# takahiroharada/OCLRadixSort

Hardware: AMD Instinct MI355X
Metric: Gkeys/s on uniform-random u32 keys; achieved % of HBM-read roofline (higher is better)
Workload: dtype u32; 1 GPU; Key-only RadixSort32, 67108864 uniform-random u32 keys (splitmix64 hi32, seed 123+step), 1xMI355X, in place; keys_per_gpu=67108864, parallelism=1 GPU, sort_algo=auto, digit_bits=8

## Files before the change

oclradixsort_amd/csrc/adlhip.hip:

```cpp
#include "../../include/adlhip.h"

#include <hip/hip_runtime.h>

#include <algorithm>
#include <cmath>
#include <cstdarg>
#include <cstdio>
#include <cstdlib>
#include <cstring>
#include <map>
#include <mutex>
#include <utility>
#include <string>
#include <vector>

#include "radix_kernels.hpp"
#include "onesweep_kernels.hpp"
#include "hybrid_kernels.hpp"
#include "persist_kernels.hpp"
#include "finish16_kernels.hpp"
#include "soa_wide_kernels.hpp"
#include "typed_kernels.hpp"

#ifndef ADLHIP_SINGLE_TU
#define X(...) extern template __global__ __VA_ARGS__;
#include "finish_kernels.inc"
#include "wavefinish_kernels.inc"
#include "passes_kernels.inc"
#include "perdigit_kernels.inc"
#undef X
#endif

namespace {

thread_local char g_err[512] = "";

int fail(const char* fmt, ...)
{
    va_list ap;
    va_start(ap, fmt);
    vsnprintf(g_err, sizeof(g_err), fmt, ap);
    va_end(ap);
    if (getenv("ADLHIP_VERBOSE")) fprintf(stderr, "[adlhip] error: %s\n", g_err);
    return ADLHIP_FAILURE;
}

#define HIPCHK(expr)                                                                           \
    do {                                                                                       \
        hipError_t _e = (expr);                                                                \
        if (_e != hipSuccess)                                                                  \
            return fail("%s failed: %s (%s:%d)", #expr, hipGetErrorString(_e), __FILE__, __LINE__); \
    } while (0)

struct ProfEntry {
    uint64_t launches = 0;
    double total_ms = 0.0;
};
struct PendingProf {
    const char* name;
    hipEvent_t e0, e1;
};
struct Staging {
    void* hptr;
    size_t bytes;
    hipEvent_t done;
    size_t capacity;
};
struct PinnedBlock {
    void* hptr;
    size_t capacity;
};
constexpr size_t kPinnedPoolMax = size_t(512) << 20;

}

struct adlhip_event {
    hipEvent_t ev;
};

struct adlhip_device {
    int idx = 0;
    hipStream_t stream = nullptr;
    bool own_stream = true;
    hipDeviceProp_t prop;
    uint64_t used_bytes = 0;
    int sort_algo = -1;
    int digit_bits = 8;
    int profile = 0;
    int tile_variant = -1;
    int rank_mode = 1;
    int lds_ordered = 0;
    int resident_wgs_device = 0;
    int resident_wgs = 0;
    int mid_path = 1;
    int mid_skip = 0;
    int mid2_skip = 0;
    int mid_backoff = 32, mid2_backoff = 64;
    int bin_finish = 1;
    int persist = 1;
    int msd2_path = 1;
    int net_lookback = 1;
    int partition_lookback = 1;
    int dict_path = 1;
    adlhip::DictBlock* d_dict = nullptr;
    uint32_t* d_msd2 = nullptr;
    std::vector<PendingProf> pending;
    std::vector<hipEvent_t> event_pool;
    std::map<std::string, ProfEntry> prof;
    std::vector<std::string> prof_order;
    std::vector<Staging> staging;
    std::vector<PinnedBlock> pinned_pool;
    size_t pinned_pool_bytes = 0;
    uint32_t* d_fault = nullptr;
    uint32_t* h_fault = nullptr;
    hipEvent_t fault_snap = nullptr;
    uint32_t* d_mid_hist = nullptr;
};

namespace {

int bind(adlhip_device* d)
{
    if (!d) return fail("null device handle");
    HIPCHK(hipSetDevice(d->idx));
    return ADLHIP_SUCCESS;
}

hipEvent_t take_event(adlhip_device* d)
{
    if (!d->event_pool.empty()) {
        hipEvent_t e = d->event_pool.back();
        d->event_pool.pop_back();
        return e;
    }
    hipEvent_t e = nullptr;
    if (hipEventCreate(&e) != hipSuccess) return nullptr;
    return e;
}

inline int trace_level()
{
    static const int level = getenv("ADLHIP_TRACE") ? atoi(getenv("ADLHIP_TRACE")) : 0;
    return level;
}

template <typename F>
int launch(adlhip_device* d, const char* name, F&& f)
{
    hipEvent_t e0 = nullptr, e1 = nullptr;
    if (d->profile) {
        e0 = take_event(d);
        e1 = take_event(d);
        if (!e0 || !e1) return fail("hipEventCreate failed");
        HIPCHK(hipEventRecord(e0, d->stream));
    }
    static const int trace = trace_level();
    if (trace) fprintf(stderr, "[adlhip] launch %s\n", name), fflush(stderr);
    f();
    hipError_t e = hipGetLastError();
    if (e != hipSuccess) return fail("launch of %s failed: %s", name, hipGetErrorString(e));
    if (trace == 1 && (e = hipStreamSynchronize(d->stream)) != hipSuccess) return fail("%s: %s", name, hipGetErrorString(e));
    if (d->profile) {
        HIPCHK(hipEventRecord(e1, d->stream));
        d->pending.push_back({name, e0, e1});
    }
    return ADLHIP_SUCCESS;
}

int fold_profile(adlhip_device* d)
{
    if (d->pending.empty()) return ADLHIP_SUCCESS;
    HIPCHK(hipStreamSynchronize(d->stream));
    for (auto& p : d->pending) {
        float ms = 0.f;
        HIPCHK(hipEventElapsedTime(&ms, p.e0, p.e1));
        auto it = d->prof.find(p.name);
        if (it == d->prof.end()) {
            d->prof_order.push_back(p.name);
            it = d->prof.emplace(p.name, ProfEntry()).first;
        }
        it->second.launches++;
        it->second.total_ms += ms;
// ... 868 lines not shown
    if (total > region_bytes || (size_t)passes * rows * 256 * 4 >= (size_t(1) << 31)) return os;
    os.ctrl = reinterpret_cast<adlhip::u32x4*>(region);
    os.tables = reinterpret_cast<adlhip::PassTable*>(region + off_tables);
    os.joint = reinterpret_cast<uint32_t*>(region + off_joint);
    os.part = reinterpret_cast<uint32_t*>(region + off_part);
    os.status = reinterpret_cast<uint32_t*>(region + off_status);
    os.rows = (uint32_t)rows;
    os.hist_wgs = wgs;
    os.per_wg = per_wg;
    os.slice0 = per_wg * wgs_per_slice;
    return os;
}

Msd2Layout msd2_layout(size_t n, size_t elem_bytes, int headroom_pct = kFullHeadroomPct)
{
    Msd2Layout L;
    const uint32_t tile = elem_bytes == 4 ? 16384u : 8192u;
    static const int env_pct = getenv("ADLHIP_SLAB_A_HEADROOM_PCT") ? atoi(getenv("ADLHIP_SLAB_A_HEADROOM_PCT")) : -1;
    if (headroom_pct == kFullHeadroomPct && env_pct >= 0) headroom_pct = env_pct;
    L.stride_a = (uint32_t)align_up(n / 256 + (n / 256) * (size_t)headroom_pct / 100 + 4096, 64);
    L.seg_shift = msd2_seg_shift(n, elem_bytes == 8);
    L.slots = 256u << L.seg_shift;
    const bool fine = elem_bytes == 4 && L.seg_shift == 8;
    L.stride_b = msd2_stride_b(n, L.slots, fine);
    L.tier_b = msd2_tier_b(n, L.slots, fine);
    L.tiles_per_bucket = (L.stride_a + tile - 1) / tile;
    L.off_mode = 0;
    L.off_cnt = L.off_mode + 256;
    L.off_off = L.off_cnt + 65536 * 4;
    L.off_hard = align_up(L.off_off + 65537 * 4, 256);
    L.off_coop = L.off_hard + 65536 * 4;
    L.off_slab_a = align_up(L.off_coop + kNetTableBytes, 256);
    L.off_slab_b = align_up(L.off_slab_a + (size_t)256 * L.stride_a * elem_bytes, 256);
    const size_t slab_b_bytes = (size_t)L.slots * L.stride_b * (elem_bytes == 4 && L.seg_shift == 8 ? 2 : elem_bytes);
    L.slab_b_in_tmp = elem_bytes == 4 && L.seg_shift == 8 && n >= kSlabInTmpMin && slab_b_bytes <= n * elem_bytes;
    L.total = L.off_slab_b + (L.slab_b_in_tmp ? 0 : slab_b_bytes);
    return L;
}

template <typename E, typename S, bool SOA = false>
int launch_large_finish(adlhip_device* d, const E* slab_b, E* out, uint32_t* out_vals, uint32_t* seg_off, uint32_t* seg_cnt, uint32_t stride_b,
                        uint32_t tier_b, uint32_t* mode, uint32_t* hard, int low_bits_max, bool bin, uint32_t seg_shift = 8);
bool use_bin_finish(const adlhip_device* d, size_t elem_bytes, bool key64, size_t n, bool whole_keys);

template <typename E>
int msd2_sort(adlhip_device* d, E* data, E* tmp, void* work, size_t n, int headroom_pct = kFullHeadroomPct)
{
    constexpr int K = sizeof(E) == 4 ? 32 : 16;
    constexpr int KEY_BITS = 8 * (int)sizeof(E);
    constexpr bool k32 = sizeof(E) == 4;
    uint32_t* cur_a = d->d_msd2;
    uint32_t* cur_b = d->d_msd2 + 8192;
    uint32_t* flag = d->d_msd2 + 8192 + 65536;
    uint32_t* done = flag + 1;
    uint32_t* sample = flag + 8;
    const Msd2Layout L = msd2_layout(n, sizeof(E), headroom_pct);
    char* wb = reinterpret_cast<char*>(work);
    uint32_t* mode = reinterpret_cast<uint32_t*>(wb + L.off_mode);
    uint32_t* seg_cnt = reinterpret_cast<uint32_t*>(wb + L.off_cnt);
    uint32_t* seg_off = reinterpret_cast<uint32_t*>(wb + L.off_off);
    E* slab_a = reinterpret_cast<E*>(wb + L.off_slab_a);
    E* slab_b = L.slab_b_in_tmp ? tmp : reinterpret_cast<E*>(wb + L.off_slab_b);
    using CT = adlhip::TileCfg<E, 8, 512, K>;
    auto kern = adlhip::msd_bucket_scatter_kernel<E, 512, K, 1>;
    auto kern2 = adlhip::msd_bucket_scatter_kernel<E, 512, K, 2>;
    if (ensure_lds(kern, CT::LDS_BYTES) || ensure_lds(kern2, CT::LDS_BYTES)) return ADLHIP_FAILURE;
    int rc = launch(d, "msd2_sample", [&] {
        hipLaunchKernelGGL(adlhip::msd2_sample_kernel<E>, dim3(adlhip::kSampleWGs), dim3(64), 0, d->stream, (const E*)data, (uint32_t)n,
                           sample, flag + 2, d->d_fault, flag, sample_dup_threshold(n));
    });
    if (rc) return rc;
    adlhip::BucketPass<E> pa;
    pa.src = data; pa.dst = slab_a; pa.cursors = cur_a; pa.cursor_shift = 5; pa.src_count_shift = 0; pa.flag = flag;
    pa.src_counts = nullptr; pa.n = (uint32_t)n;
    pa.src_stride = 0; pa.tiles_per_bucket = 1; pa.dst_stride = L.stride_a; pa.dst_total = 256u * L.stride_a; pa.start_bit = KEY_BITS - 8;
    pa.zero_me = nullptr; pa.sample = sample; pa.which_digit = 1; pa.dst16 = 0;
    pa.place = nullptr; pa.status_a = nullptr; pa.pieces = 0; pa.rows_per_chain_a = 0; pa.slice = 0; pa.seg_shift = 8;
    const uint32_t tiles_a = (uint32_t)((n + CT::TILE - 1) / CT::TILE);
    const bool slab16 = sizeof(E) == 4 && L.seg_shift == 8;
    const bool persist = d->persist && (size_t)256 * L.stride_a * sizeof(E) < (size_t(1) << 32) - (1u << 20) &&
                         (size_t)L.slots * L.stride_b * (slab16 ? 2 : sizeof(E)) < (size_t(1) << 32) - (1u << 20);
    using PC = adlhip::PersistCfg<E, 512, K>;
    const uint32_t pgrid = (uint32_t)(2 * d->prop.multiProcessorCount + 7) / 8 * 8;
    if (persist) {
        auto pk = adlhip::msd_scatter_persist_kernel<E, 512, K, 1, 4, false, 2, 0>;
        if (ensure_lds(pk, PC::LDS_BYTES)) return ADLHIP_FAILURE;
        rc = launch(d, k32 ? "msd2_pass1_u32" : "msd2_pass1_u64", [&] { hipLaunchKernelGGL(pk, dim3(pgrid), dim3(512), PC::LDS_BYTES, d->stream, pa); });
    } else {
        rc = launch(d, k32 ? "msd2_pass1_u32" : "msd2_pass1_u64", [&] { hipLaunchKernelGGL(kern, dim3(tiles_a), dim3(512), CT::LDS_BYTES, d->stream, pa); });
    }
    if (rc) return rc;
    adlhip::BucketPass<E> pb = pa;
    pb.src = slab_a; pb.dst = slab_b; pb.cursors = cur_b; pb.cursor_shift = 0; pb.src_count_shift = 5; pb.flag = flag;
    pb.src_counts = cur_a; pb.n = (uint32_t)n;
    pb.src_stride = L.stride_a; pb.tiles_per_bucket = L.tiles_per_bucket; pb.dst_stride = L.stride_b;
    pb.dst_total = L.slots * L.stride_b; pb.start_bit = KEY_BITS - 16; pb.zero_me = nullptr;
    pb.sample = sample; pb.which_digit = 2; pb.seg_shift = L.seg_shift;
    pb.dst16 = slab16 ? 1 : 0;
    if (persist) {
        auto pk16 = adlhip::msd_scatter_persist_kernel<E, 512, K, 2, 4, true, 2, 0>;
        auto pkE = adlhip::msd_scatter_persist_kernel<E, 512, K, 2, 4, false, 2, 0>;
        if (ensure_lds(pk16, PC::LDS_BYTES) || ensure_lds(pkE, PC::LDS_BYTES)) return ADLHIP_FAILURE;
        rc = launch(d, k32 ? "msd2_pass2_u32" : "msd2_pass2_u64", [&] {
            if (slab16) hipLaunchKernelGGL(pk16, dim3(pgrid), dim3(512), PC::LDS_BYTES, d->stream, pb);
            else hipLaunchKernelGGL(pkE, dim3(pgrid), dim3(512), PC::LDS_BYTES, d->stream, pb);
        });
    } else {
        rc = launch(d, k32 ? "msd2_pass2_u32" : "msd2_pass2_u64", [&] {
            hipLaunchKernelGGL(kern2, dim3(256 * L.tiles_per_bucket), dim3(512), CT::LDS_BYTES, d->stream, pb);
        });
    }
    if (rc) return rc;
    uint32_t* bar = done + 1;
    uint32_t* ctable = reinterpret_cast<uint32_t*>(wb + L.off_coop);
    using CC = adlhip::TileCfg<E, 8, 512, K>;
    auto ko = adlhip::msd2_offsets_kernel<E, 512, K>;
    if (ensure_lds(ko, CC::LDS_BYTES)) return ADLHIP_FAILURE;
    rc = launch(d, "msd2_offsets", [&] {
        hipLaunchKernelGGL(ko, dim3(net_wgs(d)), dim3(512), CC::LDS_BYTES, d->stream, cur_a, cur_b, flag, done, bar,
                           seg_cnt, seg_off, mode, (uint32_t)n, sample, data, tmp, ctable, d->d_fault, KEY_BITS,
                           8u - L.seg_shift, d->dict_path ? d->d_dict : nullptr, net_stats(d),
                           net_onesweep_args(d, wb + L.off_slab_a, (size_t)256 * L.stride_a * sizeof(E), n, 4, CC::TILE));
    });
    if (rc) return rc;
    using S = typename std::conditional<sizeof(E) == 4, uint16_t, E>::type;
    uint32_t* hard = reinterpret_cast<uint32_t*>(wb + L.off_hard);
    const int low_max = KEY_BITS - 8 - (int)L.seg_shift;
    const bool bin = use_bin_finish(d, sizeof(E), sizeof(E) == 8, L.seg_shift < 8 ? (size_t(24) << 20) : n, true);
    if (sizeof(E) == 4 && !slab16)
        return launch_large_finish<E, E>(d, slab_b, data, nullptr, seg_off, seg_cnt, L.stride_b, L.tier_b, mode, hard, low_max, bin, L.seg_shift);
    return launch_large_finish<E, S>(d, slab_b, data, nullptr, seg_off, seg_cnt, L.stride_b, L.tier_b, mode, hard, low_max, bin, L.seg_shift);
}

constexpr size_t kMsd2sAutoMin = size_t(1) << 20;
constexpr size_t kMsd2sMax = (size_t(1) << 28) + (size_t(1) << 22);
constexpr uint32_t msd2s_tile(size_t elem_bytes) { return elem_bytes == 8 ? 8192u : 16384u; }

struct Msd2sLayout {
    size_t off_mode, off_place, off_cnt, off_off, off_hard, off_coop, off_tickets, off_status_a, off_status_b, off_slab_a, off_slab_b, total;
    uint32_t pieces, slice, rows_a, rows_b, stride_a, stride_b, tier_b, ticket_words, seg_shift, slots;
    size_t status_bytes_a, status_bytes_b;
    bool slab_b_in_tmp;
};

Msd2sLayout msd2s_layout(size_t n, size_t elem_bytes = 8, bool slab16 = false, bool lean = false)
{
    Msd2sLayout L;
    const uint32_t kMsd2sTile = msd2s_tile(elem_bytes);
    double best = 1e30;
    for (uint32_t p : {16u}) {
        const size_t slice = align_up((n + p - 1) / p, kMsd2sTile);
        const size_t mean = slice / 256;
        size_t sd = 1;
        while (sd * sd < mean) ++sd;
        const size_t stride = align_up(mean + (lean ? 0 : mean / 2) + 8 * sd + 64, 64);
        const double waste = (double)((stride + kMsd2sTile - 1) / kMsd2sTile) * kMsd2sTile / (double)mean;
        if (waste < best - 1e-9) {
            best = waste;
            L.pieces = p;
            L.slice = (uint32_t)slice;
            L.stride_a = (uint32_t)stride;
        }
    }
    L.rows_a = L.slice / kMsd2sTile;
    L.rows_b = (uint32_t)(((size_t)L.pieces * L.stride_a + kMsd2sTile - 1) / kMsd2sTile);
    L.seg_shift = slab16 ? 8u : msd2_seg_shift(n, false);
    L.slots = 256u << L.seg_shift;
    L.stride_b = msd2_stride_b(n, L.slots, slab16, lean);
    L.tier_b = msd2_tier_b(n, L.slots, slab16);
    L.ticket_words = (32 + 256) * adlhip::kTicketStride;
    L.status_bytes_a = (size_t)L.pieces * L.rows_a * 1024;
    L.status_bytes_b = (size_t)256 * L.rows_b * 1024;
    L.off_mode = 0;
    L.off_place = 128;
    L.off_cnt = 256;
    L.off_off = L.off_cnt + 65536 * 4;
    L.off_hard = align_up(L.off_off + 65537 * 4, 256);
    L.off_coop = L.off_hard + 65536 * 4;
    L.off_tickets = align_up(L.off_coop + kNetTableBytes, 256);
    size_t sdb = 1;
    while (sdb * sdb * 4096 < n) ++sdb;
    const size_t bucket_bound = n / 256 + (lean ? 0 : n / 512) + 24 * (32 + 16 + 8 * (sdb + 1) + 128);
    const size_t rows_a_bound = n / kMsd2sTile + 24;
    const size_t rows_b_bound = bucket_bound / kMsd2sTile + 25;
// ... 1322 lines not shown
        });
        if (rc) return rc;
        rc = launch(d, "scan_partials", [&] {
            hipLaunchKernelGGL(adlhip::scan_single_kernel, dim3(1), dim3(adlhip::kScanNT), 0, d->stream,
                               (const uint32_t*)partial, partial, blocks, d_total);
        });
        if (rc) return rc;
        rc = launch(d, "scan_apply", [&] {
            hipLaunchKernelGGL(adlhip::scan_apply_kernel, dim3((uint32_t)blocks), dim3(adlhip::kScanNT), 0, d->stream,
                               src, dst, (const uint32_t*)partial, n);
        });
        if (rc) return rc;
    }
    if (h_sum) HIPCHK(hipMemcpyAsync(h_sum, d_total, 4, hipMemcpyDeviceToHost, d->stream));
    return ADLHIP_SUCCESS;
}


int adlhip_partition_msb_u32(adlhip_device* d, const uint32_t* in, uint32_t* out, uint32_t* counts, void* work,
                             size_t work_bytes, size_t n, int num_buckets)
{
    return partition_msb<uint32_t>(d, in, out, counts, work, work_bytes, n, num_buckets);
}

int adlhip_partition_msb_kv32(adlhip_device* d, const void* in, void* out, uint32_t* counts, void* work, size_t work_bytes,
                              size_t n, int num_buckets)
{
    return partition_msb<uint64_t>(d, static_cast<const uint64_t*>(in), static_cast<uint64_t*>(out), counts, work, work_bytes, n,
                                   num_buckets);
}

int adlhip_partition_top_byte_u32(adlhip_device* d, const uint32_t* in, uint32_t* out, uint32_t* totals256, void* work,
                                  size_t work_bytes, size_t n)
{
    return partition_top_byte_entry<uint32_t>(d, in, out, totals256, work, work_bytes, n);
}

int adlhip_partition_top_byte_kv32(adlhip_device* d, const void* in, void* out, uint32_t* totals256, void* work,
                                   size_t work_bytes, size_t n)
{
    return partition_top_byte_entry<uint64_t>(d, static_cast<const uint64_t*>(in), static_cast<uint64_t*>(out), totals256, work,
                                              work_bytes, n);
}


int adlhip_generate_keys(adlhip_device* d, int elem_kind, void* dptr, size_t n, uint64_t seed, uint64_t first_index)
{
    if (bind(d)) return ADLHIP_FAILURE;
    if (elem_kind < ADLHIP_ELEM_U32 || elem_kind > ADLHIP_ELEM_U64) return fail("bad element kind %d", elem_kind);
    if (n == 0) return ADLHIP_SUCCESS;
    if (!dptr) return fail("null buffer");
    const uint64_t base = seed * 0x9E3779B97F4A7C15ull + first_index;
    const int grid = (int)std::min<size_t>((n + 255) / 256, (size_t)d->prop.multiProcessorCount * 16);
    return launch(d, "generate_keys", [&] {
        hipLaunchKernelGGL(adlhip::generate_keys_kernel, dim3(grid), dim3(256), 0, d->stream, dptr, n, base, first_index, elem_kind);
    });
}


int adlhip_set_param(adlhip_device* d, const char* name, int value)
{
    if (!d || !name) return fail("null argument");
    if (!strcmp(name, "sort.algo")) {
        if (value < -1 || value > 1) return fail("sort.algo must be -1, 0 or 1");
        d->sort_algo = value;
    } else if (!strcmp(name, "sort.digit_bits")) {
        if (value != 4 && value != 7 && value != 8) return fail("sort.digit_bits must be 4, 7 or 8");
        d->digit_bits = value;
    } else if (!strcmp(name, "sort.tile")) {
        if (value < -1 || value >= kNumVariants) return fail("sort.tile must be in [-1,%d)", kNumVariants);
        d->tile_variant = value;

    } else if (!strcmp(name, "sort.mid")) {
        if (value < 0 || value > 3) return fail("sort.mid must be 0 (off), 1 (on), 2 (keys: always the two-launch form) or 3 (always the three-launch form)");
        d->mid_path = value;
    } else if (!strcmp(name, "sort.msd2")) {
        if (value < 0 || value > 5)
            return fail("sort.msd2 must be 0 (off), 1 (on), 2 (always, from 1 Mi elements; forms by size), 3 (always the stable passes), "
                        "4 (always the cursor passes for whole keys) or 5 (always the hybrid form for whole keys)");
        d->msd2_path = value;
    } else if (!strcmp(name, "sort.persist")) {
        if (value != 0 && value != 1) return fail("sort.persist must be 0 (one tile per workgroup, round 3) or 1 (persistent prefetching passes + 16-bit finish)");
        d->persist = value;
    } else if (!strcmp(name, "sort.net_lookback")) {
        d->net_lookback = value ? 1 : 0;
    } else if (!strcmp(name, "partition.lookback")) {
        d->partition_lookback = value ? 1 : 0;
    } else if (!strcmp(name, "sort.dict")) {
        if (value != 0 && value != 1) return fail("sort.dict must be 0 (off) or 1 (counting sort for keys that take few distinct values)");
        d->dict_path = value;
    } else if (!strcmp(name, "sort.binfinish")) {
        if (value < 0 || value > 2) return fail("sort.binfinish must be 0 (LSD finish), 1 (binning finish for whole u64 keys from 24 Mi keys up) or 2 (always, u32 keys too)");
        d->bin_finish = value;
    } else if (!strcmp(name, "debug.resident_wgs")) {
        if (value < 0) return fail("debug.resident_wgs must be >= 0");
        d->resident_wgs = value ? value : d->resident_wgs_device;
    } else if (!strcmp(name, "debug.idle_poke")) {
        const int region = (int)((uint32_t)value >> 24);
        const uint32_t word = (uint32_t)value & 0xffffffu;
        if (region < 1 || region > kIdleRegions || word >= idle_region_words(region))
            return fail("debug.idle_poke: no word %u in region %d (region << 24 | word; regions 1 d_msd2, 2 d_mid_hist, 3 d_dict, 4 d_fault)", word, region);
        if (bind(d)) return ADLHIP_FAILURE;
        hipLaunchKernelGGL(idle_poke_kernel, dim3(1), dim3(1), 0, d->stream, idle_region_base(d, region) + word);
        HIPCHK(hipGetLastError());
    } else if (!strcmp(name, "sort.rank")) {
        if (value != 0 && value != 1) return fail("sort.rank must be 0 or 1");
        if (value == 1 && !d->lds_ordered) return fail("sort.rank = 1 needs lane-ordered DS atomics; the device self-test failed");
        d->rank_mode = value;
    } else if (!strcmp(name, "profile")) {
        if (bind(d)) return ADLHIP_FAILURE;
        if (!value && fold_profile(d)) return ADLHIP_FAILURE;
        d->profile = value ? 1 : 0;
    } else {
        return fail("unknown parameter '%s'", name);
    }
    return ADLHIP_SUCCESS;
}

int adlhip_get_param(adlhip_device* d, const char* name, int* value)
{
    if (!d || !name || !value) return fail("null argument");
    if (!strcmp(name, "sort.algo")) *value = d->sort_algo;
    else if (!strcmp(name, "sort.digit_bits")) *value = d->digit_bits;
    else if (!strcmp(name, "sort.tile")) *value = d->tile_variant;
    else if (!strcmp(name, "sort.rank")) *value = d->rank_mode;
    else if (!strcmp(name, "sort.mid")) *value = d->mid_path;
    else if (!strcmp(name, "sort.msd2")) *value = d->msd2_path;
    else if (!strcmp(name, "sort.binfinish")) *value = d->bin_finish;
    else if (!strcmp(name, "sort.persist")) *value = d->persist;
    else if (!strcmp(name, "sort.dict")) *value = d->dict_path;
    else if (!strcmp(name, "partition.lookback")) *value = d->partition_lookback;
    else if (!strcmp(name, "sort.net_lookback")) *value = d->net_lookback;
    else if (!strcmp(name, "debug.resident_wgs")) *value = d->resident_wgs;
    else if (!strcmp(name, "stat.net_runs") || !strcmp(name, "stat.net_counting")) {
        uint32_t v[2] = {0u, 0u};
        HIPCHK(hipMemcpyAsync(v, net_stats(d), 8, hipMemcpyDeviceToHost, d->stream));
        HIPCHK(hipStreamSynchronize(d->stream));
        *value = (int)v[name[9] == 'c' ? 1 : 0];
    }
    else if (!strcmp(name, "debug.idle_dirty") || !strcmp(name, "debug.idle_first")) {
        uint32_t dirty = 0u, first = 0u;
        if (idle_check(d, &dirty, &first)) return ADLHIP_FAILURE;
        *value = (int)(name[11] == 'd' ? dirty : first);
    }
    else if (!strncmp(name, "debug.net_stamp", 15) && name[15] >= '0' && name[15] <= '9' && !name[16]) {
        uint32_t v = 0u;
        HIPCHK(hipMemcpyAsync(&v, net_stats(d) + 4 + (name[15] - '0'), 4, hipMemcpyDeviceToHost, d->stream));
        HIPCHK(hipStreamSynchronize(d->stream));
        *value = (int)(v & 0x7fffffffu);
    }
    else if (!strcmp(name, "sort.lds_ordered")) *value = d->lds_ordered;
    else if (!strcmp(name, "profile")) *value = d->profile;
    else return fail("unknown parameter '%s'", name);
    return ADLHIP_SUCCESS;
}


int adlhip_event_create(adlhip_device* d, adlhip_event** out)
{
    if (bind(d)) return ADLHIP_FAILURE;
    if (!out) return fail("null out pointer");
    adlhip_event* e = new adlhip_event();
    if (hipEventCreate(&e->ev) != hipSuccess) {
        delete e;
        return fail("hipEventCreate failed");
    }
    *out = e;
    return ADLHIP_SUCCESS;
}

int adlhip_event_record(adlhip_device* d, adlhip_event* ev)
{
    if (bind(d)) return ADLHIP_FAILURE;
    if (!ev) return fail("null event");
    HIPCHK(hipEventRecord(ev->ev, d->stream));
    return ADLHIP_SUCCESS;
}

int adlhip_event_elapsed_ms(adlhip_device* d, adlhip_event* a, adlhip_event* b, float* ms)
{
    if (bind(d)) return ADLHIP_FAILURE;
    if (!a || !b || !ms) return fail("null argument");
    HIPCHK(hipEventSynchronize(b->ev));
    HIPCHK(hipEventElapsedTime(ms, a->ev, b->ev));
    return ADLHIP_SUCCESS;
}

int adlhip_event_synchronize(adlhip_device* d, adlhip_event* ev)
{
    if (bind(d)) return ADLHIP_FAILURE;
    if (!ev) return fail("null event");
    HIPCHK(hipEventSynchronize(ev->ev));
    return ADLHIP_SUCCESS;
}

int adlhip_event_query(adlhip_device* d, adlhip_event* ev, int* done)
{
    if (bind(d)) return ADLHIP_FAILURE;
    if (!ev || !done) return fail("null argument");
    const hipError_t e = hipEventQuery(ev->ev);
    if (e != hipSuccess && e != hipErrorNotReady) return fail("hipEventQuery failed: %s", hipGetErrorString(e));
    (void)hipGetLastError();
    *done = e == hipSuccess ? 1 : 0;
    return ADLHIP_SUCCESS;
}

int adlhip_event_destroy(adlhip_device* d, adlhip_event* ev)
{
    if (bind(d)) return ADLHIP_FAILURE;
    if (!ev) return ADLHIP_SUCCESS;
    hipEventDestroy(ev->ev);
    delete ev;
// ... 116 lines not shown
```

oclradixsort_amd/csrc/passes_kernels.inc:

```
X(void adlhip::msd2_offsets_kernel<unsigned int, 512, 32>(unsigned int*, unsigned int*, unsigned int*, unsigned int*, unsigned int*, unsigned int*, unsigned int*, unsigned int*, unsigned int, unsigned int*, unsigned int*, unsigned int*, unsigned int*, unsigned int*, int, unsigned int, adlhip::DictBlock*, unsigned int*, adlhip::OsNet))
X(void adlhip::msd2_offsets_kernel<unsigned long, 512, 16>(unsigned int*, unsigned int*, unsigned int*, unsigned int*, unsigned int*, unsigned int*, unsigned int*, unsigned int*, unsigned int, unsigned int*, unsigned long*, unsigned long*, unsigned int*, unsigned int*, int, unsigned int, adlhip::DictBlock*, unsigned int*, adlhip::OsNet))
X(void adlhip::msd2s_offsets_kernel<unsigned int, 16384, 512, 32, 1, 4>(unsigned int const*, unsigned int, unsigned int, unsigned int, unsigned int const*, unsigned int, unsigned int, unsigned int*, unsigned int*, unsigned int*, unsigned int*, unsigned int*, unsigned int*, unsigned int, adlhip::StablePlace const*, unsigned int*, unsigned int*, unsigned int*, unsigned int*, unsigned int*, unsigned int*, unsigned int*, unsigned int, adlhip::DictBlock*, unsigned int*, adlhip::OsNet))
X(void adlhip::msd2s_offsets_kernel<unsigned long, 8192, 512, 16, 0, 4>(unsigned int const*, unsigned int, unsigned int, unsigned int, unsigned int const*, unsigned int, unsigned int, unsigned int*, unsigned int*, unsigned int*, unsigned int*, unsigned int*, unsigned int*, unsigned int, adlhip::StablePlace const*, unsigned long*, unsigned long*, unsigned int*, unsigned int*, unsigned int*, unsigned int*, unsigned int*, unsigned int, adlhip::DictBlock*, unsigned int*, adlhip::OsNet))
X(void adlhip::msd2s_offsets_kernel<unsigned long, 8192, 512, 16, 1, 4>(unsigned int const*, unsigned int, unsigned int, unsigned int, unsigned int const*, unsigned int, unsigned int, unsigned int*, unsigned int*, unsigned int*, unsigned int*, unsigned int*, unsigned int*, unsigned int, adlhip::StablePlace const*, unsigned long*, unsigned long*, unsigned int*, unsigned int*, unsigned int*, unsigned int*, unsigned int*, unsigned int, adlhip::DictBlock*, unsigned int*, adlhip::OsNet))
X(void adlhip::msd2s_offsets_kernel<unsigned long, 8192, 512, 16, 1, 8>(unsigned int const*, unsigned int, unsigned int, unsigned int, unsigned int const*, unsigned int, unsigned int, unsigned int*, unsigned int*, unsigned int*, unsigned int*, unsigned int*, unsigned int*, unsigned int, adlhip::StablePlace const*, unsigned long*, unsigned long*, unsigned int*, unsigned int*, unsigned int*, unsigned int*, unsigned int*, unsigned int, adlhip::DictBlock*, unsigned int*, adlhip::OsNet))
X(void adlhip::msd_bucket_scatter_kernel<unsigned int, 256, 16, 0>(adlhip::BucketPass<unsigned int>))
X(void adlhip::msd_bucket_scatter_kernel<unsigned int, 512, 32, 1>(adlhip::BucketPass<unsigned int>))
X(void adlhip::msd_bucket_scatter_kernel<unsigned int, 512, 32, 2>(adlhip::BucketPass<unsigned int>))
X(void adlhip::msd_bucket_scatter_kernel<unsigned int, 512, 32, 3>(adlhip::BucketPass<unsigned int>))
X(void adlhip::msd_bucket_scatter_kernel<unsigned long, 512, 16, 1>(adlhip::BucketPass<unsigned long>))
X(void adlhip::msd_bucket_scatter_kernel<unsigned long, 512, 16, 2>(adlhip::BucketPass<unsigned long>))
X(void adlhip::msd_bucket_scatter_kernel<unsigned long, 512, 16, 3>(adlhip::BucketPass<unsigned long>))
X(void adlhip::msd_lookback_scatter_kernel<unsigned int, 512, 32, false, 1>(adlhip::LookbackPass<unsigned int>))
X(void adlhip::msd_lookback_scatter_kernel<unsigned long, 512, 16, false, 0>(adlhip::LookbackPass<unsigned long>))
X(void adlhip::msd_lookback_scatter_kernel<unsigned long, 512, 16, false, 1>(adlhip::LookbackPass<unsigned long>))
X(void adlhip::msd_lookback_scatter_kernel<unsigned long, 512, 16, true, 1>(adlhip::LookbackPass<unsigned long>))
X(void adlhip::msd_scatter_persist_kernel<unsigned int, 512, 32, 1, 4, false, 2, 0>(adlhip::BucketPass<unsigned int>))
X(void adlhip::msd_scatter_persist_kernel<unsigned int, 512, 32, 2, 4, false, 2, 0>(adlhip::BucketPass<unsigned int>))
X(void adlhip::msd_scatter_persist_kernel<unsigned int, 512, 32, 2, 4, true, 2, 0>(adlhip::BucketPass<unsigned int>))
X(void adlhip::msd_scatter_persist_kernel<unsigned long, 512, 16, 1, 4, false, 2, 0>(adlhip::BucketPass<unsigned long>))
X(void adlhip::msd_scatter_persist_kernel<unsigned long, 512, 16, 2, 4, false, 2, 0>(adlhip::BucketPass<unsigned long>))
X(void adlhip::msd_scatter_persist_kernel<unsigned long, 512, 16, 2, 4, true, 2, 0>(adlhip::BucketPass<unsigned long>))
```

oclradixsort_amd/csrc/persist_kernels.hpp:

```cpp
#pragma once
#include <hip/hip_runtime.h>
#include <stdint.h>

#include "hybrid_kernels.hpp"

namespace adlhip {

template <typename E, int NT, int K>
struct PersistCfg {
    static constexpr int NW = NT / 64;
    static constexpr int TILE = NT * K;
    static constexpr int VEC = 16 / (int)sizeof(E);
    static_assert(K % VEC == 0, "whole 16-byte loads");
    static_assert(TILE <= 65536, "16-bit tile positions");
    static constexpr size_t OFF_ELEMS = 0;
    static constexpr size_t OFF_WCNT = sizeof(E) * TILE;
    static constexpr size_t OFF_WPOS = OFF_WCNT + sizeof(uint32_t) * NW * 256;
    static constexpr size_t OFF_GOFF = OFF_WPOS + sizeof(uint16_t) * NW * 256;
    static constexpr size_t OFF_PREF = OFF_GOFF + sizeof(uint32_t) * 256;
    static constexpr size_t OFF_BCNT = OFF_PREF + sizeof(uint32_t) * 260;
    static constexpr size_t OFF_WSUM = OFF_BCNT + sizeof(uint32_t) * 256;
    static constexpr size_t LDS_BYTES = OFF_WSUM + 64;
};

struct PersistTile {
    uint32_t base;
    uint32_t valid;
    uint32_t cursor_base;
};

template <typename E, int B>
__device__ __forceinline__ void rank_batch(const E* e, uint32_t* rnk, uint32_t* my_wcnt, int start_bit)
{
    const uint32_t dg0 = digit_of<8>(e[0], start_bit);
    const uint32_t d0 = (uint32_t)__builtin_amdgcn_readfirstlane((int)dg0);
    bool same = false;
    if (__all(dg0 == d0)) {
        same = true;
#pragma unroll
        for (int j = 1; j < B; ++j) same &= digit_of<8>(e[j], start_bit) == d0;
    }
    const uint32_t left = (uint32_t)__builtin_amdgcn_update_dpp((int)~dg0, (int)dg0, 0x111, 0xf, 0xf, false);
    const bool few_runs = __popcll(__ballot(left != dg0)) <= 8;
    const bool dominant = __popcll(__ballot(dg0 == d0)) >= 40;
    const int peel = few_runs ? 4 : (dominant ? 1 : 0);
    if (__all(same)) {
        uint32_t old = 0u;
        if (lane_id() == 0) old = __hip_atomic_fetch_add(&my_wcnt[d0], (uint32_t)(64 * B), __ATOMIC_RELAXED, __HIP_MEMORY_SCOPE_WORKGROUP);
        old = (uint32_t)__builtin_amdgcn_readfirstlane((int)old);
#pragma unroll
        for (int j = 0; j < B; ++j) rnk[j] = old + (uint32_t)(j * 64 + lane_id());
    } else if (peel) {
#pragma unroll
        for (int j = 0; j < B; ++j) {
            const uint32_t d = digit_of<8>(e[j], start_bit);
            uint64_t todo = __ballot(true);
            uint32_t r = 0u;
#pragma unroll 1
            for (int it = 0; it < peel && todo; ++it) {
                const uint64_t m0 = few_runs ? todo : __ballot(d == d0);
                if (!m0) break;
                const int lead = __builtin_ctzll(m0);
                const uint32_t dl = (uint32_t)__builtin_amdgcn_readlane((int)d, lead);
                const uint64_t m = __ballot(d == dl);
                uint32_t old = 0u;
                if (lane_id() == lead)
                    old = __hip_atomic_fetch_add(&my_wcnt[dl], (uint32_t)__popcll(m), __ATOMIC_RELAXED, __HIP_MEMORY_SCOPE_WORKGROUP);
                old = (uint32_t)__builtin_amdgcn_readlane((int)old, lead);
                if (d == dl) r = old + mbcnt64(m);
                todo &= ~m;
            }
            if ((todo >> lane_id()) & 1ull) r = __hip_atomic_fetch_add(&my_wcnt[d], 1u, __ATOMIC_RELAXED, __HIP_MEMORY_SCOPE_WORKGROUP);
            rnk[j] = r;
        }
    } else {
#pragma unroll
        for (int j = 0; j < B; ++j)
            rnk[j] = __hip_atomic_fetch_add(&my_wcnt[digit_of<8>(e[j], start_bit)], 1u, __ATOMIC_RELAXED, __HIP_MEMORY_SCOPE_WORKGROUP);
    }
}

template <typename E, int NT, int K, int PASS, int WPE, bool D16, int LAUX = 0, int SAUX = 0>
__global__ __launch_bounds__(NT, WPE) void msd_scatter_persist_kernel(BucketPass<E> a)
{
    using C = PersistCfg<E, NT, K>;
    constexpr int NW = C::NW;
    constexpr int TILE = C::TILE;
    constexpr int VEC = C::VEC;
    constexpr int Q = K / VEC;
    extern __shared__ __attribute__((aligned(16))) unsigned char smem[];
    E* __restrict__ s_elems = reinterpret_cast<E*>(smem + C::OFF_ELEMS);
    uint32_t* __restrict__ s_wcnt = reinterpret_cast<uint32_t*>(smem + C::OFF_WCNT);
    uint32_t* __restrict__ s_goff = reinterpret_cast<uint32_t*>(smem + C::OFF_GOFF);
    uint32_t* __restrict__ s_pref = reinterpret_cast<uint32_t*>(smem + C::OFF_PREF);
    uint32_t* __restrict__ s_bcnt = reinterpret_cast<uint32_t*>(smem + C::OFF_BCNT);
    const int tid = (int)threadIdx.x;
    const int lane = tid & 63;
    const int w = tid >> 6;
    if (a.zero_me && blockIdx.x == 0 && tid == 0) __hip_atomic_store(a.zero_me, 0u, __ATOMIC_RELAXED, __HIP_MEMORY_SCOPE_AGENT);

    uint32_t* __restrict__ s_give = reinterpret_cast<uint32_t*>(smem + C::OFF_WSUM);
    {
        if (tid == 0) s_give[8] = large_sort_gave_up(a.flag);
        __syncthreads();
        if (s_give[8]) return;
        __syncthreads();
    }
    int start_bit = a.start_bit;
    Msd2Placement place{0, 0ull};
    if (a.sample) {
        place = msd2_placement(a.sample);
        start_bit = place.top - 8 * a.which_digit;
    }
    if constexpr (PASS >= 2) start_bit += 8 - (int)a.seg_shift;

    const uint32_t G = gridDim.x, g = blockIdx.x;
    uint32_t ticket, t_end, t_step, t_origin = 0u;
    if constexpr (PASS == 1) {
        ticket = g;
        t_end = (a.n + (uint32_t)TILE - 1u) / (uint32_t)TILE;
        t_step = G;
    } else {
        uint32_t* s_wsum = reinterpret_cast<uint32_t*>(smem + C::OFF_WSUM);
        uint32_t tiles = 0u;
        if (tid < 256) {
            const uint32_t b = (((uint32_t)tid & 31u) << 3) | ((uint32_t)tid >> 5);
            uint32_t cnt = a.src_counts[b << a.src_count_shift];
            if (cnt > a.src_stride) cnt = a.src_stride;
            s_bcnt[tid] = cnt;
            tiles = (cnt + (uint32_t)TILE - 1u) / (uint32_t)TILE;
        }
        uint32_t total;
        const uint32_t ex = block_excl_scan_u32<NT>(tiles, s_wsum, &total);
        if (tid < 256) s_pref[tid] = ex;
        if (tid == 0) s_pref[256] = total;
        __syncthreads();
        const uint32_t x = g & 7u;
        t_origin = 32u * x;
        ticket = s_pref[t_origin] + (g >> 3);
        t_end = s_pref[t_origin + 32u];
        t_step = G >> 3;
    }
    if (ticket >= t_end) return;

    auto tile_of = [&](uint32_t t) -> PersistTile {
        PersistTile r;
        if constexpr (PASS == 1) {
            r.base = t * (uint32_t)TILE;
            const uint32_t left = a.n - r.base;
            r.valid = left < (uint32_t)TILE ? left : (uint32_t)TILE;
            r.cursor_base = 0u;
        } else {
            uint32_t p = t_origin;
#pragma unroll
            for (uint32_t s = 16u; s >= 1u; s >>= 1)
                if (s_pref[p + s] <= t) p += s;
            const uint32_t b = ((p & 31u) << 3) | (p >> 5);
            const uint32_t off = (t - s_pref[p]) * (uint32_t)TILE;
            const uint32_t room = s_bcnt[p] - off;
            r.base = b * a.src_stride + off;
            r.valid = room < (uint32_t)TILE ? room : (uint32_t)TILE;
            r.cursor_base = b * 256u;
        }
        return r;
    };
    const uint32_t wbase0 = (uint32_t)(w * 64 * K + lane * VEC);
    auto load_tile = [&](const PersistTile& t, E(&e)[K]) {
        uint32_t wbase = wbase0;
        asm volatile("" : "+v"(wbase));
        const __amdgpu_buffer_rsrc_t r = __builtin_amdgcn_make_buffer_rsrc(const_cast<E*>(a.src + (size_t)t.base), 0,
                                                                           (int)(t.valid * (uint32_t)sizeof(E)), 0x00020000);
        const int off = (int)(wbase * (uint32_t)sizeof(E));
#pragma unroll
        for (int q = 0; q < Q; ++q) {
            const u32x4 v = __builtin_amdgcn_raw_buffer_load_b128(r, off, q * 64 * 16, LAUX);
            if constexpr (VEC == 4) {
                e[q * 4 + 0] = v.x; e[q * 4 + 1] = v.y; e[q * 4 + 2] = v.z; e[q * 4 + 3] = v.w;
            } else {
                e[q * 2 + 0] = (E)v.x | ((E)v.y << 32);
                e[q * 2 + 1] = (E)v.z | ((E)v.w << 32);
            }
        }
    };

    uint32_t* my_wcnt = s_wcnt + w * 256;
    uint16_t* __restrict__ my_wpos = reinterpret_cast<uint16_t*>(smem + C::OFF_WPOS) + w * 256;
    constexpr uint32_t SC = D16 ? 2u : (uint32_t)sizeof(E);
    const __amdgpu_buffer_rsrc_t dst_rsrc = __builtin_amdgcn_make_buffer_rsrc(a.dst, 0, (int)(a.dst_total * SC), 0x00020000);

    E cur[K], nxt[K];
    PersistTile tc = tile_of(ticket), tn{0u, 0u, 0u};
    load_tile(tc, cur);
#pragma unroll
    for (int j = 0; j < K; ++j) asm volatile("" : "+v"(cur[j]));
    uint32_t flag_prev = 0u;
    for (;;) {
        const uint32_t ticket_n = ticket + t_step;
        const bool has_next = ticket_n < t_end;
        const uint32_t flag_now = __hip_atomic_load(a.flag, __ATOMIC_RELAXED, __HIP_MEMORY_SCOPE_AGENT);
        if (has_next) {
            tn = tile_of(ticket_n);
            load_tile(tn, nxt);
        }
        const uint32_t valid = tc.valid;
        const bool full = valid == (uint32_t)TILE;
        uint32_t tid_v = (uint32_t)tid;
        asm volatile("" : "+v"(tid_v));
        const uint32_t wbase = (tid_v >> 6) * (uint32_t)(64 * K) + (tid_v & 63u) * (uint32_t)VEC;
        const int rem = (int)valid - (int)wbase;
        if (PASS == 1 && a.sample && place.top < (int)(8 * sizeof(E))) {
            const E pre = (E)place.prefix;
            E bad = E(0);
#pragma unroll
            for (int q = 0; q < Q; ++q)
#pragma unroll
                for (int c = 0; c < VEC; ++c)
                    if (full || q * 64 * VEC + c < rem) bad |= (cur[q * VEC + c] >> place.top) ^ pre;
            if (bad != E(0)) __hip_atomic_fetch_or(a.flag, 1u, __ATOMIC_RELAXED, __HIP_MEMORY_SCOPE_AGENT);
        }
#pragma unroll
        for (int b = lane; b < 256; b += 64) my_wcnt[b] = 0u;
        uint32_t rnk2[(K + 1) / 2];
        if (full) {
            constexpr int B = 8;
            static_assert(K % B == 0, "whole batches");
#pragma unroll
            for (int j0 = 0; j0 < K; j0 += B) {
                uint32_t rnk[B];
                rank_batch<E, B>(cur + j0, rnk, my_wcnt, start_bit);
#pragma unroll
                for (int j = 0; j < B; j += 2) rnk2[(j0 + j) >> 1] = rnk[j] | (rnk[j + 1] << 16);
            }
        } else {
#pragma unroll
            for (int j = 0; j < K; j += 2) {
                uint32_t r0 = 0u, r1 = 0u;
                if ((j / VEC) * 64 * VEC + (j % VEC) < rem)
                    r0 = __hip_atomic_fetch_add(&my_wcnt[digit_of<8>(cur[j], start_bit)], 1u, __ATOMIC_RELAXED, __HIP_MEMORY_SCOPE_WORKGROUP);
                if (((j + 1) / VEC) * 64 * VEC + ((j + 1) % VEC) < rem)
                    r1 = __hip_atomic_fetch_add(&my_wcnt[digit_of<8>(cur[j + 1], start_bit)], 1u, __ATOMIC_RELAXED, __HIP_MEMORY_SCOPE_WORKGROUP);
                rnk2[j >> 1] = r0 | (r1 << 16);
            }
        }
#pragma unroll
        for (int j = 0; j < (K + 1) / 2; ++j) asm volatile("" : "+v"(rnk2[j]));
        if (lane == 0) s_give[w] = flag_prev;
        lds_barrier();
        {
            const u32x4 g0 = *reinterpret_cast<const u32x4*>(s_give), g1 = *reinterpret_cast<const u32x4*>(s_give + 4);
            static_assert(NW <= 8, "one word per wave");
            uint32_t any = 0u;
            if (NW > 0) any |= g0.x; if (NW > 1) any |= g0.y; if (NW > 2) any |= g0.z; if (NW > 3) any |= g0.w;
            if (NW > 4) any |= g1.x; if (NW > 5) any |= g1.y; if (NW > 6) any |= g1.z; if (NW > 7) any |= g1.w;
            if (any) break;
        }
        u32x4 cnt4 = {0u, 0u, 0u, 0u};
        u32x4 toff4 = {0u, 0u, 0u, 0u};
        {
            u32x4 pre4 = {0u, 0u, 0u, 0u};
#pragma unroll
            for (int i = 0; i < NW; ++i) {
                const u32x4 r = *reinterpret_cast<const u32x4*>(s_wcnt + i * 256 + 4 * lane);
                cnt4 += r;
                if (i < w) pre4 += r;
            }
            const uint32_t s4 = cnt4.x + cnt4.y + cnt4.z + cnt4.w;
            const uint32_t ex = wave_incl_scan_u32(s4) - s4;
            toff4.x = ex;
            toff4.y = ex + cnt4.x;
            toff4.z = toff4.y + cnt4.y;
            toff4.w = toff4.z + cnt4.z;
            const u32x4 p4 = toff4 + pre4;
            typedef uint32_t u32x2 __attribute__((ext_vector_type(2)));
            const u32x2 packed = {p4.x | (p4.y << 16), p4.z | (p4.w << 16)};
            *reinterpret_cast<u32x2*>(my_wpos + 4 * lane) = packed;
        }
        u32x4 at4 = {0u, 0u, 0u, 0u};
        if (w == 0) {
            uint32_t* cp = a.cursors + ((size_t)(tc.cursor_base + 4u * (uint32_t)lane) << a.cursor_shift);
            const size_t step = (size_t)1 << a.cursor_shift;
            if (cnt4.x) at4.x = __hip_atomic_fetch_add(cp + 0 * step, cnt4.x, __ATOMIC_RELAXED, __HIP_MEMORY_SCOPE_AGENT);
            if (cnt4.y) at4.y = __hip_atomic_fetch_add(cp + 1 * step, cnt4.y, __ATOMIC_RELAXED, __HIP_MEMORY_SCOPE_AGENT);
            if (cnt4.z) at4.z = __hip_atomic_fetch_add(cp + 2 * step, cnt4.z, __ATOMIC_RELAXED, __HIP_MEMORY_SCOPE_AGENT);
            if (cnt4.w) at4.w = __hip_atomic_fetch_add(cp + 3 * step, cnt4.w, __ATOMIC_RELAXED, __HIP_MEMORY_SCOPE_AGENT);
        }
        {
            constexpr int CH = K < 8 ? K : 8;
#pragma unroll
            for (int j0 = 0; j0 < K; j0 += CH) {
                uint32_t pos[CH];
#pragma unroll
                for (int j = 0; j < CH; ++j) pos[j] = my_wpos[digit_of<8>(cur[(j0 + j < K) ? j0 + j : K - 1], start_bit)];
#pragma unroll
                for (int j = 0; j < CH; ++j) {
                    const int jj = j0 + j;
                    if (jj < K) {
                        const uint32_t r = (rnk2[jj >> 1] >> (16 * (jj & 1))) & 0xffffu;
                        if (full || (jj / VEC) * 64 * VEC + (jj % VEC) < rem) s_elems[pos[j] + r] = cur[jj];
                    }
                }
            }
        }
        asm volatile("" : "+v"(at4.x), "+v"(at4.y), "+v"(at4.z), "+v"(at4.w));
        if (w == 0) {
            const bool over = (at4.x + cnt4.x > a.dst_stride) | (at4.y + cnt4.y > a.dst_stride) | (at4.z + cnt4.z > a.dst_stride) |
                              (at4.w + cnt4.w > a.dst_stride);
            if (over) __hip_atomic_fetch_or(a.flag, 1u, __ATOMIC_RELAXED, __HIP_MEMORY_SCOPE_AGENT);
            uint32_t d0 = tc.cursor_base + 4u * (uint32_t)lane;
            if constexpr (PASS >= 2)
                d0 = ((tc.cursor_base >> 8) << a.seg_shift) + ((4u * (uint32_t)lane) & ((1u << a.seg_shift) - 1u));
            u32x4 go;
            go.x = (d0 + 0u) * a.dst_stride + at4.x - toff4.x;
            go.y = (d0 + 1u) * a.dst_stride + at4.y - toff4.y;
            go.z = (d0 + 2u) * a.dst_stride + at4.z - toff4.z;
            go.w = (d0 + 3u) * a.dst_stride + at4.w - toff4.w;
            *reinterpret_cast<u32x4*>(s_goff + 4 * lane) = go * SC;
        }
        lds_barrier();
        {
            const uint32_t tsc = tid_v * SC;
            constexpr int WCH = K < 8 ? K : 8;
#pragma unroll
            for (int i0 = 0; i0 < K; i0 += WCH) {
                E v[WCH];
                uint32_t off[WCH];
#pragma unroll
                for (int i = 0; i < WCH; ++i) v[i] = s_elems[tid_v + (uint32_t)((i0 + i) * NT)];
#pragma unroll
                for (int i = 0; i < WCH; ++i) {
                    off[i] = s_goff[digit_of<8>(v[i], start_bit)] + tsc + (uint32_t)((i0 + i) * NT) * SC;
                    if (tid_v + (uint32_t)((i0 + i) * NT) >= valid) off[i] = 0xfffffff0u;
                }
#pragma unroll
                for (int i = 0; i < WCH; ++i) {
                    if constexpr (D16) {
                        __builtin_amdgcn_raw_buffer_store_b16((uint16_t)v[i], dst_rsrc, (int)off[i], 0, SAUX);
                    } else if constexpr (sizeof(E) == 4) {
                        __builtin_amdgcn_raw_buffer_store_b32((uint32_t)v[i], dst_rsrc, (int)off[i], 0, SAUX);
                    } else {
                        typedef uint32_t u32x2_t __attribute__((ext_vector_type(2)));
                        const u32x2_t t2 = {(uint32_t)v[i], (uint32_t)((uint64_t)v[i] >> 32)};
                        __builtin_amdgcn_raw_buffer_store_b64(t2, dst_rsrc, (int)off[i], 0, SAUX);
                    }
                }
                asm volatile("" ::: "memory");
            }
        }
        if (!has_next) break;
        flag_prev = flag_now;
#pragma unroll
        for (int j = 0; j < K; ++j) {
            cur[j] = nxt[j];
            asm volatile("" : "+v"(cur[j]));
        }
        tc = tn;
        ticket = ticket_n;
    }
}

}
```

Before: 207.0 Gkeys/s.

## Pack first MSD slab to 3 bytes per u32 key

In the large u32 MSD sort, pass 1 now writes only the low 24 bits of each key into the intermediate slab, since the top byte is already implied by the bucket. Each key goes out as one 16-bit store plus one 8-bit store at odd or even alignment. Pass 2 reads the packed slab with 96-bit buffer loads and unpacks four keys from every three words. This cuts slab write and read traffic by a quarter, at the cost of two narrow stores per key, which may merge poorly, and extra unpack ALU work.

```diff
diff --git a/oclradixsort_amd/csrc/adlhip.hip b/oclradixsort_amd/csrc/adlhip.hip
--- a/oclradixsort_amd/csrc/adlhip.hip
+++ b/oclradixsort_amd/csrc/adlhip.hip
@@ -98,6 +98,7 @@
     int mid_backoff = 32, mid2_backoff = 64;
     int bin_finish = 1;
     int persist = 1;
+    int slab24 = 1;
     int msd2_path = 1;
     int net_lookback = 1;
     int partition_lookback = 1;
@@ -1132,8 +1133,12 @@
                          (size_t)L.slots * L.stride_b * (slab16 ? 2 : sizeof(E)) < (size_t(1) << 32) - (1u << 20);
     using PC = adlhip::PersistCfg<E, 512, K>;
     const uint32_t pgrid = (uint32_t)(2 * d->prop.multiProcessorCount + 7) / 8 * 8;
+    const bool slab24 = slab16 && persist && d->slab24;
     if (persist) {
         auto pk = adlhip::msd_scatter_persist_kernel<E, 512, K, 1, 4, false, 2, 0>;
+        if constexpr (k32) {
+            if (slab24) pk = adlhip::msd_scatter_persist_kernel<E, 512, K, 1, 4, false, 2, 0, true, false>;
+        }
         if (ensure_lds(pk, PC::LDS_BYTES)) return ADLHIP_FAILURE;
         rc = launch(d, k32 ? "msd2_pass1_u32" : "msd2_pass1_u64", [&] { hipLaunchKernelGGL(pk, dim3(pgrid), dim3(512), PC::LDS_BYTES, d->stream, pa); });
     } else {
@@ -1150,6 +1155,9 @@
     if (persist) {
         auto pk16 = adlhip::msd_scatter_persist_kernel<E, 512, K, 2, 4, true, 2, 0>;
         auto pkE = adlhip::msd_scatter_persist_kernel<E, 512, K, 2, 4, false, 2, 0>;
+        if constexpr (k32) {
+            if (slab24) pk16 = adlhip::msd_scatter_persist_kernel<E, 512, K, 2, 4, true, 2, 0, false, true>;
+        }
         if (ensure_lds(pk16, PC::LDS_BYTES) || ensure_lds(pkE, PC::LDS_BYTES)) return ADLHIP_FAILURE;
         rc = launch(d, k32 ? "msd2_pass2_u32" : "msd2_pass2_u64", [&] {
             if (slab16) hipLaunchKernelGGL(pk16, dim3(pgrid), dim3(512), PC::LDS_BYTES, d->stream, pb);
@@ -2638,6 +2646,9 @@
     } else if (!strcmp(name, "sort.persist")) {
         if (value != 0 && value != 1) return fail("sort.persist must be 0 (one tile per workgroup, round 3) or 1 (persistent prefetching passes + 16-bit finish)");
         d->persist = value;
+    } else if (!strcmp(name, "sort.slab24")) {
+        if (value != 0 && value != 1) return fail("sort.slab24 must be 0 (the first slab of the large u32 sort holds whole keys) or 1 (3 bytes per key)");
+        d->slab24 = value;
     } else if (!strcmp(name, "sort.net_lookback")) {
         d->net_lookback = value ? 1 : 0;
     } else if (!strcmp(name, "partition.lookback")) {
@@ -2684,6 +2695,7 @@
     else if (!strcmp(name, "sort.msd2")) *value = d->msd2_path;
     else if (!strcmp(name, "sort.binfinish")) *value = d->bin_finish;
     else if (!strcmp(name, "sort.persist")) *value = d->persist;
+    else if (!strcmp(name, "sort.slab24")) *value = d->slab24;
     else if (!strcmp(name, "sort.dict")) *value = d->dict_path;
     else if (!strcmp(name, "partition.lookback")) *value = d->partition_lookback;
     else if (!strcmp(name, "sort.net_lookback")) *value = d->net_lookback;
diff --git a/oclradixsort_amd/csrc/passes_kernels.inc b/oclradixsort_amd/csrc/passes_kernels.inc
--- a/oclradixsort_amd/csrc/passes_kernels.inc
+++ b/oclradixsort_amd/csrc/passes_kernels.inc
@@ -15,9 +15,11 @@
 X(void adlhip::msd_lookback_scatter_kernel<unsigned long, 512, 16, false, 0>(adlhip::LookbackPass<unsigned long>))
 X(void adlhip::msd_lookback_scatter_kernel<unsigned long, 512, 16, false, 1>(adlhip::LookbackPass<unsigned long>))
 X(void adlhip::msd_lookback_scatter_kernel<unsigned long, 512, 16, true, 1>(adlhip::LookbackPass<unsigned long>))
-X(void adlhip::msd_scatter_persist_kernel<unsigned int, 512, 32, 1, 4, false, 2, 0>(adlhip::BucketPass<unsigned int>))
-X(void adlhip::msd_scatter_persist_kernel<unsigned int, 512, 32, 2, 4, false, 2, 0>(adlhip::BucketPass<unsigned int>))
-X(void adlhip::msd_scatter_persist_kernel<unsigned int, 512, 32, 2, 4, true, 2, 0>(adlhip::BucketPass<unsigned int>))
-X(void adlhip::msd_scatter_persist_kernel<unsigned long, 512, 16, 1, 4, false, 2, 0>(adlhip::BucketPass<unsigned long>))
-X(void adlhip::msd_scatter_persist_kernel<unsigned long, 512, 16, 2, 4, false, 2, 0>(adlhip::BucketPass<unsigned long>))
-X(void adlhip::msd_scatter_persist_kernel<unsigned long, 512, 16, 2, 4, true, 2, 0>(adlhip::BucketPass<unsigned long>))
+X(void adlhip::msd_scatter_persist_kernel<unsigned int, 512, 32, 1, 4, false, 2, 0, false, false>(adlhip::BucketPass<unsigned int>))
+X(void adlhip::msd_scatter_persist_kernel<unsigned int, 512, 32, 1, 4, false, 2, 0, true, false>(adlhip::BucketPass<unsigned int>))
+X(void adlhip::msd_scatter_persist_kernel<unsigned int, 512, 32, 2, 4, false, 2, 0, false, false>(adlhip::BucketPass<unsigned int>))
+X(void adlhip::msd_scatter_persist_kernel<unsigned int, 512, 32, 2, 4, true, 2, 0, false, false>(adlhip::BucketPass<unsigned int>))
+X(void adlhip::msd_scatter_persist_kernel<unsigned int, 512, 32, 2, 4, true, 2, 0, false, true>(adlhip::BucketPass<unsigned int>))
+X(void adlhip::msd_scatter_persist_kernel<unsigned long, 512, 16, 1, 4, false, 2, 0, false, false>(adlhip::BucketPass<unsigned long>))
+X(void adlhip::msd_scatter_persist_kernel<unsigned long, 512, 16, 2, 4, false, 2, 0, false, false>(adlhip::BucketPass<unsigned long>))
+X(void adlhip::msd_scatter_persist_kernel<unsigned long, 512, 16, 2, 4, true, 2, 0, false, false>(adlhip::BucketPass<unsigned long>))
diff --git a/oclradixsort_amd/csrc/persist_kernels.hpp b/oclradixsort_amd/csrc/persist_kernels.hpp
--- a/oclradixsort_amd/csrc/persist_kernels.hpp
+++ b/oclradixsort_amd/csrc/persist_kernels.hpp
@@ -80,14 +80,18 @@
     }
 }
 
-template <typename E, int NT, int K, int PASS, int WPE, bool D16, int LAUX = 0, int SAUX = 0>
+template <typename E, int NT, int K, int PASS, int WPE, bool D16, int LAUX = 0, int SAUX = 0, bool S24 = false, bool L24 = false>
 __global__ __launch_bounds__(NT, WPE) void msd_scatter_persist_kernel(BucketPass<E> a)
 {
+    static_assert(!(S24 || L24) || sizeof(E) == 4, "packed first slab: u32 keys");
+    static_assert(!S24 || (PASS == 1 && !D16), "pass 1 writes the packed slab");
+    static_assert(!L24 || PASS == 2, "pass 2 reads the packed slab");
     using C = PersistCfg<E, NT, K>;
     constexpr int NW = C::NW;
     constexpr int TILE = C::TILE;
     constexpr int VEC = C::VEC;
     constexpr int Q = K / VEC;
+    constexpr int KR = L24 ? Q * 3 : K;
     extern __shared__ __attribute__((aligned(16))) unsigned char smem[];
     E* __restrict__ s_elems = reinterpret_cast<E*>(smem + C::OFF_ELEMS);
     uint32_t* __restrict__ s_wcnt = reinterpret_cast<uint32_t*>(smem + C::OFF_WCNT);
@@ -165,34 +169,60 @@
         return r;
     };
     const uint32_t wbase0 = (uint32_t)(w * 64 * K + lane * VEC);
-    auto load_tile = [&](const PersistTile& t, E(&e)[K]) {
+    auto load_tile = [&](const PersistTile& t, E(&e)[KR]) {
         uint32_t wbase = wbase0;
         asm volatile("" : "+v"(wbase));
-        const __amdgpu_buffer_rsrc_t r = __builtin_amdgcn_make_buffer_rsrc(const_cast<E*>(a.src + (size_t)t.base), 0,
-                                                                           (int)(t.valid * (uint32_t)sizeof(E)), 0x00020000);
-        const int off = (int)(wbase * (uint32_t)sizeof(E));
+        constexpr uint32_t SB = L24 ? 3u : (uint32_t)sizeof(E);
+        unsigned char* src8 = reinterpret_cast<unsigned char*>(const_cast<E*>(a.src)) + (size_t)t.base * SB;
+        const __amdgpu_buffer_rsrc_t r = __builtin_amdgcn_make_buffer_rsrc(src8, 0, (int)((t.valid * SB + 3u) & ~3u), 0x00020000);
+        const int off = (int)(wbase * SB);
 #pragma unroll
         for (int q = 0; q < Q; ++q) {
-            const u32x4 v = __builtin_amdgcn_raw_buffer_load_b128(r, off, q * 64 * 16, LAUX);
-            if constexpr (VEC == 4) {
-                e[q * 4 + 0] = v.x; e[q * 4 + 1] = v.y; e[q * 4 + 2] = v.z; e[q * 4 + 3] = v.w;
+            if constexpr (L24) {
+                typedef uint32_t u32x3 __attribute__((ext_vector_type(3)));
+                const u32x3 v = __builtin_amdgcn_raw_buffer_load_b96(r, off, q * 64 * 12, LAUX);
+                e[q * 3 + 0] = v.x; e[q * 3 + 1] = v.y; e[q * 3 + 2] = v.z;
             } else {
-                e[q * 2 + 0] = (E)v.x | ((E)v.y << 32);
-                e[q * 2 + 1] = (E)v.z | ((E)v.w << 32);
+                const u32x4 v = __builtin_amdgcn_raw_buffer_load_b128(r, off, q * 64 * 16, LAUX);
+                if constexpr (VEC == 4) {
+                    e[q * 4 + 0] = v.x; e[q * 4 + 1] = v.y; e[q * 4 + 2] = v.z; e[q * 4 + 3] = v.w;
+                } else {
+                    e[q * 2 + 0] = (E)v.x | ((E)v.y << 32);
+                    e[q * 2 + 1] = (E)v.z | ((E)v.w << 32);
+                }
             }
         }
     };
 
     uint32_t* my_wcnt = s_wcnt + w * 256;
     uint16_t* __restrict__ my_wpos = reinterpret_cast<uint16_t*>(smem + C::OFF_WPOS) + w * 256;
-    constexpr uint32_t SC = D16 ? 2u : (uint32_t)sizeof(E);
+    constexpr uint32_t SC = S24 ? 3u : (D16 ? 2u : (uint32_t)sizeof(E));
     const __amdgpu_buffer_rsrc_t dst_rsrc = __builtin_amdgcn_make_buffer_rsrc(a.dst, 0, (int)(a.dst_total * SC), 0x00020000);
 
-    E cur[K], nxt[K];
+    E cur[K], nxt[KR];
+    auto take = [&](E(&r)[KR]) {
+        if constexpr (L24) {
+#pragma unroll
+            for (int j = 0; j < KR; ++j) asm volatile("" : "+v"(r[j]));
+#pragma unroll
+            for (int q = 0; q < Q; ++q) {
+                const uint32_t r0 = (uint32_t)r[q * 3 + 0], r1 = (uint32_t)r[q * 3 + 1], r2 = (uint32_t)r[q * 3 + 2];
+                cur[q * 4 + 0] = (E)(r0 & 0xffffffu);
+                cur[q * 4 + 1] = (E)((r0 >> 24) | ((r1 & 0xffffu) << 8));
+                cur[q * 4 + 2] = (E)((r1 >> 16) | ((r2 & 0xffu) << 16));
+                cur[q * 4 + 3] = (E)(r2 >> 8);
+            }
+        } else {
+#pragma unroll
+            for (int j = 0; j < K; ++j) {
+                cur[j] = r[j];
+                asm volatile("" : "+v"(cur[j]));
+            }
+        }
+    };
     PersistTile tc = tile_of(ticket), tn{0u, 0u, 0u};
-    load_tile(tc, cur);
-#pragma unroll
-    for (int j = 0; j < K; ++j) asm volatile("" : "+v"(cur[j]));
+    load_tile(tc, nxt);
+    take(nxt);
     uint32_t flag_prev = 0u;
     for (;;) {
         const uint32_t ticket_n = ticket + t_step;
@@ -277,7 +307,7 @@
         }
         u32x4 at4 = {0u, 0u, 0u, 0u};
         if (w == 0) {
-            uint32_t* cp = a.cursors + ((size_t)(tc.cursor_base + 4u * (uint32_t)lane) << a.cursor_shift);
+            uint32_t* cp = a.cursors + ((size_t)(tc.cursor_base + 4u * (tid_v & 63u)) << a.cursor_shift);
             const size_t step = (size_t)1 << a.cursor_shift;
             if (cnt4.x) at4.x = __hip_atomic_fetch_add(cp + 0 * step, cnt4.x, __ATOMIC_RELAXED, __HIP_MEMORY_SCOPE_AGENT);
             if (cnt4.y) at4.y = __hip_atomic_fetch_add(cp + 1 * step, cnt4.y, __ATOMIC_RELAXED, __HIP_MEMORY_SCOPE_AGENT);
@@ -333,7 +363,13 @@
                 }
 #pragma unroll
                 for (int i = 0; i < WCH; ++i) {
-                    if constexpr (D16) {
+                    if constexpr (S24) {
+                        const uint32_t k = (uint32_t)v[i];
+                        const uint32_t odd = off[i] & 1u;
+                        const uint32_t h = odd ? k >> 8 : k, c = odd ? k : k >> 16;
+                        __builtin_amdgcn_raw_buffer_store_b16((uint16_t)h, dst_rsrc, (int)(off[i] + odd), 0, SAUX);
+                        __builtin_amdgcn_raw_buffer_store_b8((uint8_t)c, dst_rsrc, (int)(off[i] + 2u - 2u * odd), 0, SAUX);
+                    } else if constexpr (D16) {
                         __builtin_amdgcn_raw_buffer_store_b16((uint16_t)v[i], dst_rsrc, (int)off[i], 0, SAUX);
                     } else if constexpr (sizeof(E) == 4) {
                         __builtin_amdgcn_raw_buffer_store_b32((uint32_t)v[i], dst_rsrc, (int)off[i], 0, SAUX);
@@ -348,11 +384,7 @@
         }
         if (!has_next) break;
         flag_prev = flag_now;
-#pragma unroll
-        for (int j = 0; j < K; ++j) {
-            cur[j] = nxt[j];
-            asm volatile("" : "+v"(cur[j]));
-        }
+        take(nxt);
         tc = tn;
         ticket = ticket_n;
     }
```

Result: slower. 201.2 Gkeys/s (-2.8%).
